# GZHoffie/approximate-string-matching

Measured on AMD Instinct MI355X. Metric: alignments/sec (1e6-pair batch, 100bp, err=0.10) per GPU; NW penalty bit-exact %, higher is better.
Workload: dtype u64; 1 GPU; C2: 1000000 pairs per GPU, len 100-100, err 0.10, k=3, x=o=e=1,1,1, aligners nw+leap+greedy, greedy tails=clean; pairs_per_gpu=1000000

## Files before the change

### approximate-string-matching_amd/csrc/asm_nwband.h

```cpp
#pragma once
#include <stdint.h>

#if defined(__HIPCC__)
#include <hip/hip_runtime.h>
#define NWB_HD __device__ __forceinline__
#else
#define NWB_HD inline
#endif

typedef unsigned long long nwb_u64;

#if defined(__HIPCC__)
NWB_HD int nwb_popc(uint32_t x) { return __popc(x); }
NWB_HD int nwb_popc64(nwb_u64 x) { return __popcll(x); }
NWB_HD uint32_t nwb_alignbit(uint32_t hi, uint32_t lo, uint32_t s) { return __builtin_amdgcn_alignbit(hi, lo, s); }
NWB_HD uint32_t nwb_sbfe1(uint32_t b, int r) { return (uint32_t)__builtin_amdgcn_sbfe((int)b, r, 1); }
typedef unsigned short nwb_u16x2 __attribute__((ext_vector_type(2)));
typedef short nwb_i16x2 __attribute__((ext_vector_type(2)));
NWB_HD uint32_t nwb_pk_add(uint32_t a, uint32_t b) {
    return __builtin_bit_cast(uint32_t, __builtin_bit_cast(nwb_u16x2, a) + __builtin_bit_cast(nwb_u16x2, b));
}
NWB_HD uint32_t nwb_pk_shl(uint32_t a, int s) {
    return __builtin_bit_cast(uint32_t, __builtin_bit_cast(nwb_u16x2, a) << (nwb_u16x2)((unsigned short)s));
}
NWB_HD uint32_t nwb_pk_shr(uint32_t a, int s) {
    return __builtin_bit_cast(uint32_t, __builtin_bit_cast(nwb_u16x2, a) >> (nwb_u16x2)((unsigned short)s));
}
NWB_HD uint32_t nwb_pk_sar(uint32_t a, int s) {
    return __builtin_bit_cast(uint32_t, __builtin_bit_cast(nwb_i16x2, a) >> (nwb_i16x2)((short)s));
}
#else
NWB_HD int nwb_popc(uint32_t x) { return __builtin_popcount(x); }
NWB_HD int nwb_popc64(nwb_u64 x) { return __builtin_popcountll(x); }
NWB_HD uint32_t nwb_alignbit(uint32_t hi, uint32_t lo, uint32_t s) {
    return (uint32_t)((((nwb_u64)hi << 32) | (nwb_u64)lo) >> (s & 31u));
}
NWB_HD uint32_t nwb_sbfe1(uint32_t b, int r) { return 0u - ((b >> r) & 1u); }
NWB_HD uint32_t nwb_pk_add(uint32_t a, uint32_t b) {
    return ((a & 0x7FFF7FFFu) + (b & 0x7FFF7FFFu)) ^ ((a ^ b) & 0x80008000u);
}
NWB_HD uint32_t nwb_pk_shl(uint32_t a, int s) { return (a << s) & (0x00010001u * ((0xFFFFu << s) & 0xFFFFu)); }
NWB_HD uint32_t nwb_pk_shr(uint32_t a, int s) { return (a >> s) & (0x00010001u * (0xFFFFu >> s)); }
NWB_HD uint32_t nwb_pk_sar(uint32_t a, int s) {
    const uint32_t lo = (uint32_t)((int32_t)(int16_t)(a & 0xFFFFu) >> s) & 0xFFFFu;
    const uint32_t hi = (uint32_t)((int32_t)(int16_t)(a >> 16) >> s) & 0xFFFFu;
    return lo | (hi << 16);
}
#endif

NWB_HD int nwb_band_bound(int C, int m, int nn) { return 2 * (C - 1) - (nn > m ? nn - m : m - nn); }

template <int W>
struct BandWord;
template <>
struct BandWord<32> {
    typedef uint32_t T;
};
template <>
struct BandWord<64> {
    typedef nwb_u64 T;
};

struct NoColumnSink {
    static constexpr bool kNeedsColumns = false;
    template <typename WT>
    NWB_HD void operator()(int, WT, WT) const {}
};

template <int W>
NWB_HD typename BandWord<W>::T band_text_bit(typename BandWord<W>::T b, int r);
template <>
NWB_HD uint32_t band_text_bit<32>(uint32_t b, int r) {
    return nwb_sbfe1(b, r);
}
template <>
NWB_HD nwb_u64 band_text_bit<64>(nwb_u64 b, int r) {
    return 0ull - ((b >> r) & 1ull);
}

template <int ND, int W, typename Sink = NoColumnSink>
NWB_HD int nw_band(const uint32_t (&A0)[ND + 2], const uint32_t (&A1)[ND + 2], const uint32_t (&B0)[ND],
                    const uint32_t (&B1)[ND], int m, int nn, const Sink& sink = Sink()) {
    typedef typename BandWord<W>::T WT;
    constexpr int C = W / 2;
    constexpr int NBLK = ND * 32 / W;
    constexpr WT TOP = (WT)1 << (W - 1);
#define BLK(ARR, q) (W == 32 ? (WT)ARR[(q)] : (WT)((nwb_u64)ARR[2 * (q)] | ((nwb_u64)ARR[2 * (q) + 1] << 32)))
    WT VP = ~(WT)0, VN = 0;
    int S = W;
    WT lo0 = BLK(A0, 0), lo1 = BLK(A1, 0), hi0 = 0, hi1 = 0;

#define NW_BAND_COLUMN(SLIDE, BW0, BW1, R)                                                           \
    {                                                                                                 \
        if (SLIDE) {                                                                                  \
            lo0 = (lo0 >> 1) | (hi0 << (W - 1)), hi0 >>= 1;                                           \
            lo1 = (lo1 >> 1) | (hi1 << (W - 1)), hi1 >>= 1;                                           \
            VP = (VP >> 1) | TOP, VN >>= 1;                                                           \
        }                                                                                             \
        const WT T0 = (WT)0 - (((BW0) >> (R)) & (WT)1);                                               \
        const WT T1 = (WT)0 - (((BW1) >> (R)) & (WT)1);                                               \
        const WT Eq = ~((lo0 ^ T0) | (lo1 ^ T1));                                                     \
        const WT D0 = ((((Eq & VP) + VP) ^ VP) | Eq) | VN;                                            \
        const WT HP = VN | ~(D0 | VP);                                                                \
        const WT HN = VP & D0;                                                                        \
        if (SLIDE)                                                                                    \
            S += 1 - (int)(D0 >> (W - 1));                                                            \
        else                                                                                          \
            S += (int)(HP >> (W - 1)) - (int)(HN >> (W - 1));                                         \
        const WT X = (HP << 1) | (WT)1;                                                               \
        VP = (HN << 1) | ~(D0 | X);                                                                   \
        VN = D0 & X;                                                                                  \
    }

    {
        const WT b0 = BLK(B0, 0), b1 = BLK(B1, 0);
        const int c1 = nn < C ? nn : C;
        for (int r = 0; r < c1; r++) {
            NW_BAND_COLUMN(false, b0, b1, r)
            sink(r + 1, VP, VN);
        }
    }
    if (Sink::kNeedsColumns) {
#pragma unroll
        for (int bq = 0; bq < NBLK; bq++) {
            const WT b0 = BLK(B0, bq), b1 = BLK(B1, bq);
            const int r0 = bq == 0 ? C : 0;
            int rend = nn - W * bq;
            rend = rend > W ? W : rend;
            for (int r = r0; r < rend; r++) {
                if (r == C) hi0 = BLK(A0, bq + 1), hi1 = BLK(A1, bq + 1);
                NW_BAND_COLUMN(true, b0, b1, r)
                sink(W * bq + r + 1, VP, VN);
            }
        }
    } else if (nn > C) {
        WT VPin = (VP >> 1) | TOP, VNin = VN >> 1;
#pragma unroll
        for (int bq = 0; bq < NBLK; bq++) {
            const WT b0 = BLK(B0, bq), b1 = BLK(B1, bq);
            const int r0 = bq == 0 ? C : 0;
            int rend = nn - W * bq;
            rend = rend > W ? W : rend;
            WT acc = 0;
#pragma unroll
            for (int half = 0; half < 2; half++) {
                constexpr int CB = W == 32 ? C - 1 : C;
                const int ra = half == 0 ? r0 : (r0 > CB ? r0 : CB);
                const int rb = half == 0 ? (rend < CB ? rend : CB) : rend;
                if (W != 32 && half == 1) hi0 = BLK(A0, bq + 1), hi1 = BLK(A1, bq + 1);
                const uint32_t p0l = W == 32 ? (half == 0 ? (bq > 0 ? A0[bq > 0 ? bq - 1 : 0] : 0u) : A0[bq]) : 0u;
                const uint32_t p0h = W == 32 ? (half == 0 ? A0[bq] : A0[bq + 1]) : 0u;
                const uint32_t p1l = W == 32 ? (half == 0 ? (bq > 0 ? A1[bq > 0 ? bq - 1 : 0] : 0u) : A1[bq]) : 0u;
                const uint32_t p1h = W == 32 ? (half == 0 ? A1[bq] : A1[bq + 1]) : 0u;
                const int shb = half == 0 ? W - CB : -CB;
                for (int r = ra; r < rb; r++) {
                    if (W == 32) {
                        lo0 = (WT)nwb_alignbit(p0h, p0l, (uint32_t)(r + shb));
                        lo1 = (WT)nwb_alignbit(p1h, p1l, (uint32_t)(r + shb));
                    } else {
                        lo0 = (lo0 >> 1) | (hi0 << (W - 1)), hi0 >>= 1;
                        lo1 = (lo1 >> 1) | (hi1 << (W - 1)), hi1 >>= 1;
                    }
                    const WT T0 = band_text_bit<W>(b0, r), T1 = band_text_bit<W>(b1, r);
                    const WT Eq = ~((lo0 ^ T0) | (lo1 ^ T1));
                    const WT D0 = ((((Eq & VPin) + VPin) ^ VPin) | Eq) | VNin;
                    const WT HP = VNin | ~(D0 | VPin);
                    const WT HN = VPin & D0;
                    acc = (acc << 1) | (D0 >> (W - 1));
                    const WT D0s = D0 >> 1;
                    VPin = HN | ~(D0s | HP) | TOP;
                    VNin = HP & D0s;
                }
            }
            if (rend > r0) S += (rend - r0) - (W == 32 ? nwb_popc((uint32_t)acc) : nwb_popc64((nwb_u64)acc));
        }
        VP = VPin << 1;
        VN = VNin << 1;
    }
#undef NW_BAND_COLUMN
#undef BLK
    const int top = nn > C - 1 ? nn - (C - 1) : 1;
    const int bstar = m - top;
    if (bstar < 0 || bstar > W - 1) return -1;
    const WT above = bstar == W - 1 ? (WT)0 : (~(WT)0 << (bstar + 1));
    const int up = W == 32 ? nwb_popc((uint32_t)(VP & above)) : nwb_popc64((nwb_u64)(VP & above));
    const int dn = W == 32 ? nwb_popc((uint32_t)(VN & above)) : nwb_popc64((nwb_u64)(VN & above));
    const int result = S - up + dn;
    return result <= nwb_band_bound(C, m, nn) ? result : -1;
}


template <int ND, int N>
NWB_HD uint32_t nwb_chunk2(const uint32_t (&P)[N], const uint32_t (&Q)[N], int k) {
    if (k < 0 || k >= 2 * ND) return 0u;
    const uint32_t p = P[k >> 1], q = Q[k >> 1];
    return (k & 1) ? (p >> 16) | (q & 0xFFFF0000u) : (p & 0xFFFFu) | (q << 16);
}

NWB_HD int nwb_band16_result(uint32_t vp, uint32_t vn, int S, int m, int nn) {
    constexpr int W = 16, C = 8;
    const int top = nn > C - 1 ? nn - (C - 1) : 1;
    const int bstar = m - top;
    if (bstar < 0 || bstar > W - 1) return -1;
    const uint32_t above = (0xFFFFu << (bstar + 1)) & 0xFFFFu;
    const int result = S - nwb_popc(vp & above) + nwb_popc(vn & above);
    return result <= nwb_band_bound(C, m, nn) ? result : -1;
}

template <int ND, int NA>
NWB_HD void nw_band2x16(const uint32_t (&A0p)[NA], const uint32_t (&A1p)[NA], const uint32_t (&B0p)[ND],
                        const uint32_t (&B1p)[ND], int mp, int np, const uint32_t (&A0q)[NA], const uint32_t (&A1q)[NA],
                        const uint32_t (&B0q)[ND], const uint32_t (&B1q)[ND], int mq, int nq, int& result_p, int& result_q) {
    constexpr int W = 16, C = 8, CB = C - 1;
    constexpr int NBLK = 2 * ND;
    constexpr uint32_t TOP = 0x80008000u, ONE = 0x00010001u, LOW = 0x0000FFFFu, HIGH = 0xFFFF0000u;
    const int nmin = np < nq ? np : nq, nmax = np < nq ? nq : np;
    uint32_t VP = ~0u, VN = 0u;
    int Sp = W, Sq = W;

    {
        const uint32_t lo0 = nwb_chunk2<ND>(A0p, A0q, 0), lo1 = nwb_chunk2<ND>(A1p, A1q, 0);
        const uint32_t b0 = nwb_chunk2<ND>(B0p, B0q, 0), b1 = nwb_chunk2<ND>(B1p, B1q, 0);
        uint32_t hp = 0u, hn = 0u;
        const int c1 = nmax < C ? nmax : C;
        for (int r = 0; r < c1; r++) {
            const uint32_t L = (r < np ? LOW : 0u) | (r < nq ? HIGH : 0u);
            const uint32_t T0 = nwb_pk_sar(nwb_pk_shl(b0, 15 - r), 15), T1 = nwb_pk_sar(nwb_pk_shl(b1, 15 - r), 15);
            const uint32_t Eq = ~((lo0 ^ T0) | (lo1 ^ T1));
            const uint32_t D0 = ((nwb_pk_add(Eq & VP, VP) ^ VP) | Eq) | VN;
            const uint32_t HP = VN | ~(D0 | VP);
            const uint32_t HN = VP & D0;
            hp = nwb_pk_shr(hp, 1) | (HP & TOP & L);
            hn = nwb_pk_shr(hn, 1) | (HN & TOP & L);
            const uint32_t X = nwb_pk_shl(HP, 1) | ONE;
            VP = ((nwb_pk_shl(HN, 1) | ~(D0 | X)) & L) | (VP & ~L);
            VN = ((D0 & X) & L) | (VN & ~L);
        }
        Sp += nwb_popc(hp & LOW) - nwb_popc(hn & LOW);
        Sq += nwb_popc(hp >> 16) - nwb_popc(hn >> 16);
    }

    uint32_t VPin = nwb_pk_shr(VP, 1) | TOP, VNin = nwb_pk_shr(VN, 1);
#define NW2_COLUMNS(FREEZE, RA, RB, U0, V0, U1, V1, SHB)                                                   \
    {                                                                                                       \
        const uint32_t v0s = nwb_pk_shl(V0, 1), v1s = nwb_pk_shl(V1, 1);                                    \
        for (int r = (RA); r < (RB); r++) {                                                                 \
            const int s = r + (SHB);                                                             \
            const uint32_t lo0 = nwb_pk_shr(U0, s) | nwb_pk_shl(v0s, 15 - s);                               \
            const uint32_t lo1 = nwb_pk_shr(U1, s) | nwb_pk_shl(v1s, 15 - s);                               \
            const uint32_t T0 = nwb_pk_sar(nwb_pk_shl(b0, 15 - r), 15), T1 = nwb_pk_sar(nwb_pk_shl(b1, 15 - r), 15); \
            const uint32_t Eq = ~((lo0 ^ T0) | (lo1 ^ T1));                                                 \
            const uint32_t D0 = ((nwb_pk_add(Eq & VPin, VPin) ^ VPin) | Eq) | VNin;                         \
            const uint32_t HP = VNin | ~(D0 | VPin);                                                        \
            const uint32_t HN = VPin & D0;                                                                  \
            const uint32_t D0s = nwb_pk_shr(D0, 1);                                                         \
            if (FREEZE) {                                                                                   \
                const int col = W * bq + r;                                                                 \
                const uint32_t L = (col < np ? LOW : 0u) | (col < nq ? HIGH : 0u);                          \
                acc = nwb_pk_shr(acc, 1) | (D0 & TOP & L);                                                  \
                VPin = ((HN | ~(D0s | HP) | TOP) & L) | (VPin & ~L);                                        \
                VNin = ((HP & D0s) & L) | (VNin & ~L);                                                      \
            } else {                                                                                        \
                acc = nwb_pk_shr(acc, 1) | (D0 & TOP);                                                      \
                VPin = HN | ~(D0s | HP) | TOP;                                                              \
                VNin = HP & D0s;                                                                            \
            }                                                                                               \
        }                                                                                                   \
    }
    if (nmax > C) {
#pragma unroll
        for (int bq = 0; bq < NBLK; bq++) {
            const int r0 = bq == 0 ? C : 0;
            int rend = nmax - W * bq;
            rend = rend > W ? W : rend;
            if (rend <= r0) continue;
            const uint32_t b0 = nwb_chunk2<ND>(B0p, B0q, bq), b1 = nwb_chunk2<ND>(B1p, B1q, bq);
            const uint32_t a0m = nwb_chunk2<ND>(A0p, A0q, bq - 1), a0c = nwb_chunk2<ND>(A0p, A0q, bq), a0n = nwb_chunk2<ND>(A0p, A0q, bq + 1);
            const uint32_t a1m = nwb_chunk2<ND>(A1p, A1q, bq - 1), a1c = nwb_chunk2<ND>(A1p, A1q, bq), a1n = nwb_chunk2<ND>(A1p, A1q, bq + 1);
            uint32_t acc = 0u;
            if (W * bq + W <= nmin) {
                if (r0 < CB) NW2_COLUMNS(false, r0, CB, a0m, a0c, a1m, a1c, W - CB)
                NW2_COLUMNS(false, (r0 > CB ? r0 : CB), W, a0c, a0n, a1c, a1n, -CB)
            } else {
                if (r0 < CB) NW2_COLUMNS(true, r0, (rend < CB ? rend : CB), a0m, a0c, a1m, a1c, W - CB)
                NW2_COLUMNS(true, (r0 > CB ? r0 : CB), rend, a0c, a0n, a1c, a1n, -CB)
            }
            int cp = np - W * bq, cq = nq - W * bq;
            cp = (cp > W ? W : (cp < r0 ? r0 : cp)) - r0;
            cq = (cq > W ? W : (cq < r0 ? r0 : cq)) - r0;
            Sp += cp - nwb_popc(acc & LOW);
            Sq += cq - nwb_popc(acc >> 16);
        }
    }
#undef NW2_COLUMNS
    const uint32_t VPf = nwb_pk_shl(VPin, 1), VNf = nwb_pk_shl(VNin, 1);
    result_p = nwb_band16_result(VPf & LOW, VNf & LOW, Sp, mp, np);
    result_q = nwb_band16_result(VPf >> 16, VNf >> 16, Sq, mq, nq);
}
```

### approximate-string-matching_amd/host/nw_host_check.cpp

```cpp
#include <stdint.h>
#include <string.h>

#include <vector>

#include "../csrc/asm_nwband.h"

namespace {
constexpr int ND = 4;

struct Planes {
    uint32_t a0[ND + 2], a1[ND + 2], b0[ND], b1[ND];
    int m, n;
};

void fill(uint32_t* p0, uint32_t* p1, const unsigned char* s, int len) {
    for (int q = 0; q < len; q++) {
        const int code = s[q] == 'C' ? 1 : s[q] == 'G' ? 2 : s[q] == 'T' ? 3 : 0;
        if (code & 1) p0[q >> 5] |= 1u << (q & 31);
        if (code & 2) p1[q >> 5] |= 1u << (q & 31);
    }
}

bool load(Planes& P, long i, const unsigned char* reads, const uint32_t* read_off, const unsigned char* refs, const uint32_t* ref_off) {
    memset(&P, 0, sizeof P);
    P.m = (int)(read_off[i + 1] - read_off[i]);
    P.n = (int)(ref_off[i + 1] - ref_off[i]);
    if (P.m > 32 * ND || P.n > 32 * ND) return false;
    fill(P.a0, P.a1, reads + read_off[i], P.m);
    fill(P.b0, P.b1, refs + ref_off[i], P.n);
    return true;
}
}

extern "C" int nw_host_band(long n, const unsigned char* reads, const uint32_t* read_off, const unsigned char* refs,
                            const uint32_t* ref_off, int W, int32_t* out) {
    for (long i = 0; i < n; i++) {
        Planes P;
        if (!load(P, i, reads, read_off, refs, ref_off)) return -2;
        if (W == 32)
            out[i] = nw_band<ND, 32>(P.a0, P.a1, P.b0, P.b1, P.m, P.n);
        else if (W == 64)
            out[i] = nw_band<ND, 64>(P.a0, P.a1, P.b0, P.b1, P.m, P.n);
        else
            return -1;
    }
    return 0;
}

extern "C" int nw_host_pair2(const unsigned char* reads, const uint32_t* read_off, const unsigned char* refs, const uint32_t* ref_off,
                             long k, const int64_t* ip, const int64_t* iq, int32_t* rp, int32_t* rq) {
    for (long j = 0; j < k; j++) {
        Planes P, Q;
        if (!load(P, ip[j], reads, read_off, refs, ref_off) || !load(Q, iq[j], reads, read_off, refs, ref_off)) return -2;
        int a = -1, b = -1;
        nw_band2x16<ND>(P.a0, P.a1, P.b0, P.b1, P.m, P.n, Q.a0, Q.a1, Q.b0, Q.b1, Q.m, Q.n, a, b);
        rp[j] = a, rq[j] = b;
    }
    return 0;
}

extern "C" int nw_host_full(long n, const unsigned char* reads, const uint32_t* read_off, const unsigned char* refs,
                            const uint32_t* ref_off, int32_t* out) {
    std::vector<int> row;
    for (long i = 0; i < n; i++) {
        const unsigned char* a = reads + read_off[i];
        const unsigned char* b = refs + ref_off[i];
        const int m = (int)(read_off[i + 1] - read_off[i]), nn = (int)(ref_off[i + 1] - ref_off[i]);
        row.assign((size_t)m + 1, 0);
        for (int r = 0; r <= m; r++) row[r] = r;
        for (int j = 1; j <= nn; j++) {
            int diag = row[0];
            row[0] = j;
            for (int r = 1; r <= m; r++) {
                const int sub = diag + (a[r - 1] != b[j - 1]);
                diag = row[r];
                int best = sub < row[r] + 1 ? sub : row[r] + 1;
                row[r] = best < row[r - 1] + 1 ? best : row[r - 1] + 1;
            }
        }
        out[i] = row[m];
    }
    return 0;
}
```

Baseline: 5.642 billion read pairs/s through NW+Leap+Greedy (whole job; consecutive steps overlap, inputs rotate over resident batches; value_in_order = the same steps strictly in order).

## Streamline packed 2x16 NW band inner loop with bitop3 and bit-reversed text shifts

Rewrites the inner column loop of the paired 16-lane banded Myers NW kernel. Ternary boolean ops become single v_bitop3 instructions, and the read window is built with alignbit over whole 32-bit runs instead of two packed shifts per plane. The reference characters are bit-reversed once per block so each step takes the top bit and doubles, instead of doing a shift and sign-extend pair per row. It also adds a per-block state sink and a host checker that compares block states against a scalar model. Together these aim to cut VALU instructions per DP cell, at the cost of relying on gfx950-specific bitop3 and inline asm.

```diff
diff --git a/approximate-string-matching_amd/csrc/asm_nwband.h b/approximate-string-matching_amd/csrc/asm_nwband.h
--- a/approximate-string-matching_amd/csrc/asm_nwband.h
+++ b/approximate-string-matching_amd/csrc/asm_nwband.h
@@ -29,6 +29,16 @@
 NWB_HD uint32_t nwb_pk_sar(uint32_t a, int s) {
     return __builtin_bit_cast(uint32_t, __builtin_bit_cast(nwb_i16x2, a) >> (nwb_i16x2)((short)s));
 }
+template <int TT>
+NWB_HD uint32_t nwb_bitop3(uint32_t a, uint32_t b, uint32_t c) {
+    return __builtin_amdgcn_bitop3_b32(a, b, c, TT);
+}
+NWB_HD uint32_t nwb_dbl(uint32_t x) {
+    uint32_t r;
+    asm("v_add_u32 %0, %1, %1" : "=v"(r) : "v"(x));
+    return r;
+}
+NWB_HD uint32_t nwb_brev(uint32_t x) { return __builtin_bitreverse32(x); }
 #else
 NWB_HD int nwb_popc(uint32_t x) { return __builtin_popcount(x); }
 NWB_HD int nwb_popc64(nwb_u64 x) { return __builtin_popcountll(x); }
@@ -46,7 +56,23 @@
     const uint32_t hi = (uint32_t)((int32_t)(int16_t)(a >> 16) >> s) & 0xFFFFu;
     return lo | (hi << 16);
 }
+template <int TT>
+NWB_HD uint32_t nwb_bitop3(uint32_t a, uint32_t b, uint32_t c) {
+    uint32_t r = 0u;
+    for (int i = 0; i < 8; i++)
+        if ((TT >> i) & 1) r |= ((i & 4) ? a : ~a) & ((i & 2) ? b : ~b) & ((i & 1) ? c : ~c);
+    return r;
+}
+NWB_HD uint32_t nwb_dbl(uint32_t x) { return x + x; }
+NWB_HD uint32_t nwb_brev(uint32_t x) {
+    x = ((x >> 1) & 0x55555555u) | ((x & 0x55555555u) << 1);
+    x = ((x >> 2) & 0x33333333u) | ((x & 0x33333333u) << 2);
+    x = ((x >> 4) & 0x0F0F0F0Fu) | ((x & 0x0F0F0F0Fu) << 4);
+    x = ((x >> 8) & 0x00FF00FFu) | ((x & 0x00FF00FFu) << 8);
+    return (x >> 16) | (x << 16);
+}
 #endif
+constexpr int NWB_A = 0xF0, NWB_B = 0xCC, NWB_C = 0xAA;
 
 NWB_HD int nwb_band_bound(int C, int m, int nn) { return 2 * (C - 1) - (nn > m ? nn - m : m - nn); }
 
@@ -196,6 +222,22 @@
     const uint32_t p = P[k >> 1], q = Q[k >> 1];
     return (k & 1) ? (p >> 16) | (q & 0xFFFF0000u) : (p & 0xFFFFu) | (q << 16);
 }
+template <int ND, int N>
+NWB_HD uint32_t nwb_run32(const uint32_t (&P)[N], int k) {
+    const int d = k < 0 ? -1 : k >> 1;
+    const uint32_t lo = d >= 0 && d < ND ? P[d >= 0 && d < ND ? d : 0] : 0u;
+    if (!(k & 1)) return lo;
+    const uint32_t hi = d + 1 >= 0 && d + 1 < ND ? P[d + 1 >= 0 && d + 1 < ND ? d + 1 : 0] : 0u;
+    return nwb_alignbit(hi, lo, 16);
+}
+template <int ND, int N>
+NWB_HD uint32_t nwb_low16(const uint32_t (&P)[N], int k) {
+    if (k < 0 || k >= 2 * ND) return 0u;
+    return (k & 1) ? P[k >> 1] >> 16 : P[k >> 1];
+}
+struct NoBlockSink {
+    NWB_HD void operator()(int, uint32_t, uint32_t, int, int) const {}
+};
 
 NWB_HD int nwb_band16_result(uint32_t vp, uint32_t vn, int S, int m, int nn) {
     constexpr int W = 16, C = 8;
@@ -207,10 +249,11 @@
     return result <= nwb_band_bound(C, m, nn) ? result : -1;
 }
 
-template <int ND, int NA>
+template <int ND, int NA, typename BlockSink = NoBlockSink>
 NWB_HD void nw_band2x16(const uint32_t (&A0p)[NA], const uint32_t (&A1p)[NA], const uint32_t (&B0p)[ND],
                         const uint32_t (&B1p)[ND], int mp, int np, const uint32_t (&A0q)[NA], const uint32_t (&A1q)[NA],
-                        const uint32_t (&B0q)[ND], const uint32_t (&B1q)[ND], int mq, int nq, int& result_p, int& result_q) {
+                        const uint32_t (&B0q)[ND], const uint32_t (&B1q)[ND], int mq, int nq, int& result_p, int& result_q,
+                        const BlockSink& block_sink = BlockSink()) {
     constexpr int W = 16, C = 8, CB = C - 1;
     constexpr int NBLK = 2 * ND;
     constexpr uint32_t TOP = 0x80008000u, ONE = 0x00010001u, LOW = 0x0000FFFFu, HIGH = 0xFFFF0000u;
@@ -241,31 +284,44 @@
     }
 
     uint32_t VPin = nwb_pk_shr(VP, 1) | TOP, VNin = nwb_pk_shr(VN, 1);
-#define NW2_COLUMNS(FREEZE, RA, RB, U0, V0, U1, V1, SHB)                                                   \
-    {                                                                                                       \
-        const uint32_t v0s = nwb_pk_shl(V0, 1), v1s = nwb_pk_shl(V1, 1);                                    \
-        for (int r = (RA); r < (RB); r++) {                                                                 \
-            const int s = r + (SHB);                                                             \
-            const uint32_t lo0 = nwb_pk_shr(U0, s) | nwb_pk_shl(v0s, 15 - s);                               \
-            const uint32_t lo1 = nwb_pk_shr(U1, s) | nwb_pk_shl(v1s, 15 - s);                               \
-            const uint32_t T0 = nwb_pk_sar(nwb_pk_shl(b0, 15 - r), 15), T1 = nwb_pk_sar(nwb_pk_shl(b1, 15 - r), 15); \
-            const uint32_t Eq = ~((lo0 ^ T0) | (lo1 ^ T1));                                                 \
-            const uint32_t D0 = ((nwb_pk_add(Eq & VPin, VPin) ^ VPin) | Eq) | VNin;                         \
-            const uint32_t HP = VNin | ~(D0 | VPin);                                                        \
-            const uint32_t HN = VPin & D0;                                                                  \
-            const uint32_t D0s = nwb_pk_shr(D0, 1);                                                         \
-            if (FREEZE) {                                                                                   \
-                const int col = W * bq + r;                                                                 \
-                const uint32_t L = (col < np ? LOW : 0u) | (col < nq ? HIGH : 0u);                          \
-                acc = nwb_pk_shr(acc, 1) | (D0 & TOP & L);                                                  \
-                VPin = ((HN | ~(D0s | HP) | TOP) & L) | (VPin & ~L);                                        \
-                VNin = ((HP & D0s) & L) | (VNin & ~L);                                                      \
-            } else {                                                                                        \
-                acc = nwb_pk_shr(acc, 1) | (D0 & TOP);                                                      \
-                VPin = HN | ~(D0s | HP) | TOP;                                                              \
-                VNin = HP & D0s;                                                                            \
-            }                                                                                               \
-        }                                                                                                   \
+    constexpr int TT_EQ = ~((NWB_A ^ NWB_B) | NWB_C) & 0xFF;
+    constexpr int TT_D0 = ((NWB_A ^ NWB_B) | NWB_C) & 0xFF;
+    constexpr int TT_ORN = (NWB_A | ~(NWB_B | NWB_C)) & 0xFF;
+    constexpr int TT_ACC = ((NWB_A & NWB_B) | NWB_C) & 0xFF;
+    constexpr int TT_SEL = ((NWB_A & NWB_B) | (~NWB_A & NWB_C)) & 0xFF;
+#define NW2_COLUMNS(FREEZE, RA, RB, K, SHB)                                                                      \
+    {                                                                                                             \
+        const uint32_t rp0 = nwb_run32<ND>(A0p, (K)), rp1 = nwb_run32<ND>(A1p, (K));                              \
+        const uint32_t u0 = nwb_chunk2<ND>(A0p, A0q, (K)), u1 = nwb_chunk2<ND>(A1p, A1q, (K));                    \
+        const uint32_t hq0 = nwb_low16<ND>(A0q, (K) + 1), hq1 = nwb_low16<ND>(A1q, (K) + 1);                      \
+        for (int r = (RA); r < (RB); r++) {                                                                       \
+            const int s = r + (SHB);                                                                   \
+            const uint32_t keep = (0x10000u << s) - 1u;                \
+            const uint32_t w0 = nwb_alignbit(hq0, nwb_bitop3<TT_SEL>(keep, rp0, u0), (uint32_t)s);                \
+            const uint32_t w1 = nwb_alignbit(hq1, nwb_bitop3<TT_SEL>(keep, rp1, u1), (uint32_t)s);                \
+            const uint32_t T0 = nwb_pk_sar(y0, 15), T1 = nwb_pk_sar(y1, 15);                                      \
+            y0 = nwb_dbl(y0), y1 = nwb_dbl(y1);                                                                   \
+            const uint32_t x1 = w1 ^ T1;                                                                          \
+            const uint32_t Eq = nwb_bitop3<TT_EQ>(w0, T0, x1);                                                    \
+            const uint32_t sum = nwb_pk_add(Eq & VPin, VPin);                                                     \
+            const uint32_t D0a = nwb_bitop3<TT_D0>(sum, VPin, Eq);  \
+            const uint32_t HP = nwb_bitop3<TT_ORN>(VNin, D0a, VPin);                      \
+            const uint32_t HN = VPin & D0a;                                                  \
+            const uint32_t D0s = nwb_pk_shr(D0a | VNin, 1);                                                       \
+            const uint32_t VPn = nwb_bitop3<TT_ORN>(HN, D0s, HP);       \
+            const uint32_t VNn = HP & D0s;                                                                        \
+            if (FREEZE) {                                                                                         \
+                const int col = W * bq + r;                                                                       \
+                const uint32_t L = (col < np ? LOW : 0u) | (col < nq ? HIGH : 0u);                                \
+                acc = nwb_bitop3<TT_ACC>(D0a, TOP & L, acc >> 1);       \
+                VPin = (VPn & L) | (VPin & ~L);                                                                   \
+                VNin = (VNn & L) | (VNin & ~L);                                                                   \
+            } else {                                                                                              \
+                acc = nwb_bitop3<TT_ACC>(D0a, TOP, acc >> 1);                                                     \
+                VPin = VPn;                                                                                       \
+                VNin = VNn;                                                                                       \
+            }                                                                                                     \
+        }                                                                                                         \
     }
     if (nmax > C) {
 #pragma unroll
@@ -274,22 +330,22 @@
             int rend = nmax - W * bq;
             rend = rend > W ? W : rend;
             if (rend <= r0) continue;
-            const uint32_t b0 = nwb_chunk2<ND>(B0p, B0q, bq), b1 = nwb_chunk2<ND>(B1p, B1q, bq);
-            const uint32_t a0m = nwb_chunk2<ND>(A0p, A0q, bq - 1), a0c = nwb_chunk2<ND>(A0p, A0q, bq), a0n = nwb_chunk2<ND>(A0p, A0q, bq + 1);
-            const uint32_t a1m = nwb_chunk2<ND>(A1p, A1q, bq - 1), a1c = nwb_chunk2<ND>(A1p, A1q, bq), a1n = nwb_chunk2<ND>(A1p, A1q, bq + 1);
+            uint32_t y0 = nwb_brev(nwb_chunk2<ND>(B0q, B0p, bq)) << r0;
+            uint32_t y1 = nwb_brev(nwb_chunk2<ND>(B1q, B1p, bq)) << r0;
             uint32_t acc = 0u;
             if (W * bq + W <= nmin) {
-                if (r0 < CB) NW2_COLUMNS(false, r0, CB, a0m, a0c, a1m, a1c, W - CB)
-                NW2_COLUMNS(false, (r0 > CB ? r0 : CB), W, a0c, a0n, a1c, a1n, -CB)
+                if (r0 < CB) NW2_COLUMNS(false, r0, CB, bq - 1, W - CB)
+                NW2_COLUMNS(false, (r0 > CB ? r0 : CB), W, bq, -CB)
             } else {
-                if (r0 < CB) NW2_COLUMNS(true, r0, (rend < CB ? rend : CB), a0m, a0c, a1m, a1c, W - CB)
-                NW2_COLUMNS(true, (r0 > CB ? r0 : CB), rend, a0c, a0n, a1c, a1n, -CB)
+                if (r0 < CB) NW2_COLUMNS(true, r0, (rend < CB ? rend : CB), bq - 1, W - CB)
+                NW2_COLUMNS(true, (r0 > CB ? r0 : CB), rend, bq, -CB)
             }
             int cp = np - W * bq, cq = nq - W * bq;
             cp = (cp > W ? W : (cp < r0 ? r0 : cp)) - r0;
             cq = (cq > W ? W : (cq < r0 ? r0 : cq)) - r0;
             Sp += cp - nwb_popc(acc & LOW);
             Sq += cq - nwb_popc(acc >> 16);
+            block_sink(bq, VPin, VNin, Sp, Sq);
         }
     }
 #undef NW2_COLUMNS
diff --git a/approximate-string-matching_amd/host/nw_host_check.cpp b/approximate-string-matching_amd/host/nw_host_check.cpp
--- a/approximate-string-matching_amd/host/nw_host_check.cpp
+++ b/approximate-string-matching_amd/host/nw_host_check.cpp
@@ -59,6 +59,68 @@
     return 0;
 }
 
+namespace {
+void band16_blocks(const Planes& P, int32_t* st) {
+    const auto bit = [](const uint32_t* pl, int q) -> uint16_t { return q >= 0 && q < 32 * ND ? (pl[q >> 5] >> (q & 31)) & 1u : 0u; };
+    const auto window = [&](const uint32_t* pl, int top) {
+        uint16_t w = 0;
+        for (int k = 0; k < 16; k++) w |= (uint16_t)(bit(pl, top - 1 + k) << k);
+        return w;
+    };
+    uint16_t VP = 0xFFFFu, VN = 0;
+    int S = 16;
+    for (int j = 1; j <= P.n && j <= 8; j++) {
+        const uint16_t T0 = bit(P.b0, j - 1) ? 0xFFFFu : 0, T1 = bit(P.b1, j - 1) ? 0xFFFFu : 0;
+        const uint16_t Eq = ~((window(P.a0, 1) ^ T0) | (window(P.a1, 1) ^ T1));
+        const uint16_t D0 = (uint16_t)((((uint16_t)(Eq & VP) + VP) ^ VP) | Eq | VN);
+        const uint16_t HP = VN | (uint16_t)~(D0 | VP), HN = VP & D0;
+        S += (HP >> 15) - (HN >> 15);
+        const uint16_t X = (uint16_t)(HP << 1) | 1u;
+        VP = (uint16_t)(HN << 1) | (uint16_t)~(D0 | X);
+        VN = D0 & X;
+    }
+    uint16_t VPin = (VP >> 1) | 0x8000u, VNin = VN >> 1;
+    for (int j = 9; j <= P.n; j++) {
+        const uint16_t T0 = bit(P.b0, j - 1) ? 0xFFFFu : 0, T1 = bit(P.b1, j - 1) ? 0xFFFFu : 0;
+        const uint16_t Eq = ~((window(P.a0, j - 7) ^ T0) | (window(P.a1, j - 7) ^ T1));
+        const uint16_t D0 = (uint16_t)((((uint16_t)(Eq & VPin) + VPin) ^ VPin) | Eq | VNin);
+        const uint16_t HP = VNin | (uint16_t)~(D0 | VPin), HN = VPin & D0;
+        S += 1 - (D0 >> 15);
+        const uint16_t D0s = D0 >> 1;
+        VPin = HN | (uint16_t)~(D0s | HP) | 0x8000u;
+        VNin = HP & D0s;
+        int32_t* o = st + 4 * ((j - 1) / 16);
+        o[0] = VPin, o[1] = VNin, o[2] = S, o[3] = 1;
+    }
+}
+struct BlockState {
+    int32_t* p;
+    int32_t* q;
+    void operator()(int bq, uint32_t vpin, uint32_t vnin, int sp, int sq) const {
+        p[4 * bq] = (int32_t)(vpin & 0xFFFFu), p[4 * bq + 1] = (int32_t)(vnin & 0xFFFFu), p[4 * bq + 2] = sp, p[4 * bq + 3] = 1;
+        q[4 * bq] = (int32_t)(vpin >> 16), q[4 * bq + 1] = (int32_t)(vnin >> 16), q[4 * bq + 2] = sq, q[4 * bq + 3] = 1;
+    }
+};
+}
+
+extern "C" int nw_host_pair2_blocks(const unsigned char* reads, const uint32_t* read_off, const unsigned char* refs,
+                                    const uint32_t* ref_off, long k, const int64_t* ip, const int64_t* iq, int32_t* got_p,
+                                    int32_t* got_q, int32_t* want_p, int32_t* want_q) {
+    constexpr int PER = 4 * 2 * ND;
+    memset(got_p, 0, sizeof(int32_t) * PER * k), memset(got_q, 0, sizeof(int32_t) * PER * k);
+    memset(want_p, 0, sizeof(int32_t) * PER * k), memset(want_q, 0, sizeof(int32_t) * PER * k);
+    for (long j = 0; j < k; j++) {
+        Planes P, Q;
+        if (!load(P, ip[j], reads, read_off, refs, ref_off) || !load(Q, iq[j], reads, read_off, refs, ref_off)) return -2;
+        int a = -1, b = -1;
+        const BlockState sink{got_p + PER * j, got_q + PER * j};
+        nw_band2x16<ND, ND + 2, BlockState>(P.a0, P.a1, P.b0, P.b1, P.m, P.n, Q.a0, Q.a1, Q.b0, Q.b1, Q.m, Q.n, a, b, sink);
+        band16_blocks(P, want_p + PER * j);
+        band16_blocks(Q, want_q + PER * j);
+    }
+    return 0;
+}
+
 extern "C" int nw_host_full(long n, const unsigned char* reads, const uint32_t* read_off, const unsigned char* refs,
                             const uint32_t* ref_off, int32_t* out) {
     std::vector<int> row;
```

After: 5.810 billion read pairs/s through NW+Leap+Greedy (whole job; consecutive steps overlap, inputs rotate over resident batches; value_in_order = the same steps strictly in order) (median of 6 runs). 3.0% higher.
